# xieydd/crane-scheduler

Measured on AMD Instinct MI355X. Metric: placements/sec, higher is better.
Workload: dtype f64

## Files before the change

### crane-scheduler_amd/crane_dyn/__init__.py

```python
from __future__ import annotations

import ctypes as C
import os

import numpy as np

_HERE = os.path.dirname(os.path.abspath(__file__))
LIB_PATH = os.path.join(os.path.dirname(_HERE), "lib", "libcrane_dyn.so")

CRANE_TS_INVALID = -(2**63)
CRANE_POD_DAEMONSET = 1
_ERRS = {-1: "invalid argument", -2: "HIP error", -3: "bad state", -4: "policy parse error", -5: "I/O error"}


class CraneError(RuntimeError):
    def __init__(self, code, msg):
        super().__init__(f"{_ERRS.get(code, code)}: {msg}")
        self.code = code


class _CPolicy(C.Structure):
    _fields_ = [
        ("n_sync", C.c_int32), ("sync_name", C.POINTER(C.c_char_p)), ("sync_period_ns", C.POINTER(C.c_int64)),
        ("n_pred", C.c_int32), ("pred_name", C.POINTER(C.c_char_p)), ("pred_limit", C.POINTER(C.c_double)),
# ... 74 lines not shown
        "crane_dyn_group_set_option": (C.c_int, [vp, C.c_char_p, C.c_int64]),
        "crane_dyn_group_size": (C.c_int32, [vp]),
        "crane_dyn_group_shard": (C.c_int, [vp, C.c_int32, P(C.c_int32), P(C.c_int64), P(C.c_int64)]),
        "crane_dyn_group_engine": (vp, [vp, C.c_int32, C.c_int32]),
        "crane_dyn_group_upload_nodes": (C.c_int, [vp, C.c_int64, vp, vp, vp, vp]),
        "crane_dyn_group_upload_bindings": (C.c_int, [vp, C.c_int64, vp, vp]),
        "crane_dyn_group_step_keys_async": (C.c_int, [vp, C.c_int64, C.c_int64, C.c_int64, vp, vp, vp]),
        "crane_dyn_group_sync": (C.c_int, [vp]),
        "crane_dyn_group_schedule": (C.c_int, [vp, C.c_int64, C.c_int64, C.c_int64, vp, vp, vp, vp]),
        "crane_dyn_group_step_keys_batch": (C.c_int, [vp, C.c_int32, vp, vp, C.c_int64, vp, vp, vp]),
        "crane_dyn_group_update_nodes": (C.c_int, [vp, C.c_int64, vp, vp, vp, vp, vp]),
        "crane_dyn_group_update_node_steps": (C.c_int, [vp, C.c_int64, vp, vp, vp, vp, vp, C.c_int64, C.c_int64,
                                                        vp, vp, vp, vp]),
        "crane_dyn_group_resize_nodes": (C.c_int, [vp, C.c_int64]),
        "crane_dyn_group_binding_records": (C.c_int, [vp, C.c_int64, C.c_int64]),
        "crane_dyn_group_add_bindings": (C.c_int, [vp, C.c_int64, vp, vp]),
        "crane_dyn_group_gc_bindings": (C.c_int, [vp, C.c_int64]),
        "crane_dyn_group_binding_count": (C.c_int64, [vp]),
        "crane_dyn_group_refresh_hot_values": (C.c_int, [vp, C.c_int64, C.c_int64]),
        "crane_dyn_group_hot_values": (C.c_int, [vp, C.c_int64, vp]),
        "crane_dyn_group_node_steps": (C.c_int, [vp, C.c_int64, C.c_int64, C.c_int64, vp, vp, vp, vp]),
        "crane_queue_create": (C.c_int, [C.c_int32, C.c_int32, P(vp)]),
        "crane_queue_wait": (C.c_int, [vp]),
        "crane_queue_last_error": (C.c_char_p, [vp]),
        "crane_queue_packets": (C.c_uint64, [vp]),
        "crane_queue_destroy": (C.c_int, [vp]),
        "crane_dyn_step_keys_queue": (C.c_int, [vp, C.c_int64, C.c_int64, C.c_int64, vp, vp, vp, vp]),
        "crane_dyn_forget_queue": (C.c_int, [vp, vp]),
        "crane_dyn_step_flush": (C.c_int, [vp]),
        "crane_dyn_num_predicates": (C.c_int32, [vp]),
        "crane_dyn_filter_counts_async": (C.c_int, [vp, C.c_int64, vp, vp, vp, vp]),
        "crane_dyn_filter_counts": (C.c_int, [vp, C.c_int64, vp, vp, vp]),
        "crane_dyn_group_filter_counts": (C.c_int, [vp, C.c_int64, vp, vp, vp]),
    }
    for name, (res, args) in sig.items():
        f = getattr(L, name)
        f.restype = res
        f.argtypes = args
    return L


lib = _load()

ABI_SYMBOLS = (
    "crane_policy_load_file", "crane_policy_load_bytes", "crane_policy_view", "crane_policy_free",
    "crane_tz_offset", "crane_parse_annotation", "crane_parse_annotations", "crane_dyn_create", "crane_dyn_destroy", "crane_dyn_last_error",
    "crane_dyn_num_metrics", "crane_dyn_metric_name", "crane_dyn_upload_nodes", "crane_dyn_upload_bindings",
    "crane_dyn_refresh_hot_values", "crane_dyn_eval", "crane_dyn_eval_keys_async", "crane_dyn_step_keys_async",
    "crane_dyn_refresh_hot_values_async", "crane_dyn_node_pass_async", "crane_dyn_greedy", "crane_dyn_key_node",
    "crane_dyn_set_profiling", "crane_dyn_stage_times", "crane_dyn_hot_values",
    "crane_dyn_version", "crane_dyn_binding_records", "crane_dyn_add_bindings", "crane_dyn_gc_bindings",
    "crane_dyn_binding_count", "crane_dyn_eval_compact", "crane_dyn_eval_matrix_async", "crane_dyn_set_option",
    "crane_translate_event", "crane_dyn_debug_trace", "crane_num_feasible_nodes_to_find", "crane_dyn_select",
    "crane_tz_load", "crane_tz_load_bytes", "crane_tz_free", "crane_tz_lookup", "crane_tz_date",
    "crane_parse_annotation_tz", "crane_parse_annotations_tz", "crane_dyn_step_slots", "crane_dyn_node_steps",
    "crane_dyn_node_steps_subset", "crane_dyn_update_nodes", "crane_dyn_update_node_steps",
    "crane_dyn_forget_stream", "crane_dyn_resize_nodes", "crane_shard_range", "crane_dyn_group_create", "crane_dyn_group_destroy",
    "crane_dyn_group_last_error", "crane_dyn_group_set_option", "crane_dyn_group_size", "crane_dyn_group_shard",
    "crane_dyn_group_engine", "crane_dyn_group_upload_nodes", "crane_dyn_group_upload_bindings",
    "crane_dyn_group_step_keys_async", "crane_dyn_group_sync", "crane_dyn_group_schedule",
    "crane_dyn_group_step_keys_batch", "crane_dyn_group_update_nodes", "crane_dyn_group_update_node_steps",
    "crane_dyn_group_resize_nodes", "crane_dyn_group_binding_records", "crane_dyn_group_add_bindings",
    "crane_dyn_group_gc_bindings", "crane_dyn_group_binding_count", "crane_dyn_group_refresh_hot_values",
    "crane_dyn_group_hot_values", "crane_dyn_group_node_steps",
    "crane_queue_create", "crane_queue_wait", "crane_queue_last_error", "crane_queue_destroy",
    "crane_queue_packets",
    "crane_dyn_step_keys_queue", "crane_dyn_forget_queue", "crane_dyn_step_flush",
    "crane_dyn_num_predicates", "crane_dyn_filter_counts_async", "crane_dyn_filter_counts",
    "crane_dyn_group_filter_counts",
)


def _ptr(a):
    return None if a is None else C.c_void_p(a.ctypes.data)


def num_feasible_nodes_to_find(n_nodes, percentage=0):
    return lib.crane_num_feasible_nodes_to_find(int(n_nodes), int(percentage))


class Policy:

    def __init__(self, spec):
        self.spec = {k: [tuple(x) for x in spec.get(k, [])] for k in ("syncPolicy", "predicate", "priority", "hotValue")}
        sp, pr, pi, hv = (self.spec[k] for k in ("syncPolicy", "predicate", "priority", "hotValue"))
        n = lambda xs: max(1, len(xs))
        self._keep = [
            (C.c_char_p * n(sp))(*[a.encode() for a, _ in sp]), (C.c_int64 * n(sp))(*[int(b) for _, b in sp]),
            (C.c_char_p * n(pr))(*[a.encode() for a, _ in pr]), (C.c_double * n(pr))(*[float(b) for _, b in pr]),
            (C.c_char_p * n(pi))(*[a.encode() for a, _ in pi]), (C.c_double * n(pi))(*[float(b) for _, b in pi]),
            (C.c_int64 * n(hv))(*[int(a) for a, _ in hv]), (C.c_int64 * n(hv))(*[int(b) for _, b in hv]),
        ]
        k = self._keep
        cp = C.POINTER
        self.c = _CPolicy(len(sp), C.cast(k[0], cp(C.c_char_p)), C.cast(k[1], cp(C.c_int64)),
                          len(pr), C.cast(k[2], cp(C.c_char_p)), C.cast(k[3], cp(C.c_double)),
                          len(pi), C.cast(k[4], cp(C.c_char_p)), C.cast(k[5], cp(C.c_double)),
                          len(hv), C.cast(k[6], cp(C.c_int64)), C.cast(k[7], cp(C.c_int64)))

    @staticmethod
    def _from_doc(doc):
        v = lib.crane_policy_view(doc).contents
# ... 6 lines not shown
        lib.crane_policy_free(doc)
        return Policy(spec)

    @staticmethod
    def load_bytes(data: bytes | str) -> "Policy":
        if isinstance(data, str):
            data = data.encode()
        doc, err = C.c_void_p(), C.create_string_buffer(512)
        rc = lib.crane_policy_load_bytes(data, len(data), C.byref(doc), err, len(err))
        if rc:
            raise CraneError(rc, err.value.decode())
        return Policy._from_doc(doc)

    @staticmethod
    def load_file(path: str) -> "Policy":
        doc, err = C.c_void_p(), C.create_string_buffer(512)
        rc = lib.crane_policy_load_file(path.encode(), C.byref(doc), err, len(err))
        if rc:
            raise CraneError(rc, err.value.decode())
        return Policy._from_doc(doc)


def default_policy_spec():
    m = 60 * 10**9
    return {
        "syncPolicy": [("cpu_usage_avg_5m", 3 * m), ("cpu_usage_max_avg_1h", 15 * m), ("cpu_usage_max_avg_1d", 180 * m),
                       ("mem_usage_avg_5m", 3 * m), ("mem_usage_max_avg_1h", 15 * m), ("mem_usage_max_avg_1d", 180 * m)],
        "predicate": [("cpu_usage_avg_5m", 0.65), ("cpu_usage_max_avg_1h", 0.75), ("mem_usage_avg_5m", 0.65),
                      ("mem_usage_max_avg_1h", 0.75)],
        "priority": [("cpu_usage_avg_5m", 0.2), ("cpu_usage_max_avg_1h", 0.3), ("cpu_usage_max_avg_1d", 0.5),
                     ("mem_usage_avg_5m", 0.2), ("mem_usage_max_avg_1h", 0.3), ("mem_usage_max_avg_1d", 0.5)],
        "hotValue": [(5 * m, 5), (1 * m, 2)],
    }


def tz_offset(name: str | None = None) -> int:
    off = C.c_int64()
    rc = lib.crane_tz_offset(None if name is None else name.encode(), C.byref(off))
    if rc:
        raise CraneError(rc, f"unsupported time zone {name!r}")
    return off.value


def parse_annotation(s: str, tz_offset_s: int):
    b = s.encode()
    v, t = C.c_double(), C.c_int64()
    lib.crane_parse_annotation(b, len(b), tz_offset_s, C.byref(v), C.byref(t))
    return v.value, t.value


class Zone:

    def __init__(self, name=None, zoneinfo_dir=None, tzif=None):
        h = C.c_void_p()
        if tzif is not None:
            rc = lib.crane_tz_load_bytes(tzif, len(tzif), C.byref(h))
        else:
            rc = lib.crane_tz_load((name or "").encode(), None if zoneinfo_dir is None else zoneinfo_dir.encode(),
                                   C.byref(h))
        if rc:
            raise CraneError(rc, f"time zone {name!r} not loadable")
        self.h = h

    def lookup(self, unix_s):
        off, st, en = C.c_int32(), C.c_int64(), C.c_int64()
        lib.crane_tz_lookup(self.h, int(unix_s), C.byref(off), C.byref(st), C.byref(en))
# ... 624 lines not shown
```

### crane-scheduler_amd/csrc/engine.hip

```cpp
#include <hip/hip_runtime.h>

#include <algorithm>
#include <chrono>
#include <cmath>
#include <cstdio>
#include <cstdlib>
#include <cstring>
#include <memory>
#include <mutex>
#include <string>
#include <vector>

#include "../../include/crane_dyn.h"
#include "bindings.hpp"
#include "dyn_types.hpp"
#include "kernels.hpp"

using namespace crane;

namespace {

hipError_t before_free() { return crane::tl_aql ? crane::aql_wait(crane::tl_aql) : hipSuccess; }

template <typename T>
// ... 594 lines not shown
        HIPTRY(h, launch_hot_count_large(rp.bn, h->sd->bts.p, rp.Bk, h->N, cut, gl, h->k2_sorted.p, h->buckets.p,
                                         h->n_cu, st, kK2lThreads));
        h->buckets_zero = false;
        h->buckets_dense = true;
        return CRANE_OK;
    }
    h->buckets_dense = false;
    if (!h->buckets_zero)
        if (int rc = zero_for(h, h->buckets.p, nb, st)) return rc;
    HIPTRY(h, launch_hot_count(h->sd->bnode.p, h->sd->bts.p, h->B, h->N, rp.cut, h->buckets.p, st));
    h->buckets_zero = false;
    return CRANE_OK;
}

static int hot_values_locked(crane_dyn* h, int64_t now_ns, int64_t hv_ts_ns, hipStream_t st,
                             const PodPrep* pods = nullptr, bool* pods_done = nullptr) {
    if (pods_done) *pods_done = false;
    RefreshPlan rp;
    if (int rc = refresh_plan(h, now_ns, hv_ts_ns, st, rp)) return rc;
    return refresh_launch(h, rp, st, pods, pods_done);
}

static int k1_bs(const crane_dyn* h) {
    return h->hv_from_counts && h->counts_pending && h->hx_pending ? 1 << h->hx_g.bb : kK1Block;
}

static int k1_args(crane_dyn* h, K1Args& a, uint32_t* cnt_out, const K1Step* step, bool* consume_out) {
    if (h->N < 0) return h->fail(CRANE_E_STATE, "upload nodes before the node pass");
    a = K1Args{};
    a.pol = h->dp;
    a.N = h->N;
    a.val = h->sd->val.p;
    a.ts = h->sd->ts.p;
    const bool keep = !step;
    a.out = keep ? h->rec.p : nullptr;
    a.hv_ts_counts = h->hv_ts_counts;
    const bool consume = h->hv_from_counts && h->counts_pending;
    if (cnt_out && !consume) return h->fail(CRANE_E_STATE, "per-window counts need a hot-value refresh first");
    if (consume) {
        HIPTRY(h, h->hvc.reserve((size_t)std::max<int64_t>(h->N, 1)));
        if (h->hx_pending) {
            const HotPart& g = h->hx_g;
            a.hx_region = h->k2_sorted.p;
            a.hx_CO = h->k2_sorted.p + g.cap;
            a.hx_nblk = g.nblk;
        } else if (h->dl_pending) {
            a.buckets = h->dl_adj[h->dl_cur].p;
            a.bucket_base = h->dl_zero ? h->dl_adj[h->dl_cur].p : h->dl_base.p;
            a.buckets_keep = 0;
        } else {
            a.buckets = h->buckets.p;
            a.buckets_keep = h->buckets_dense ? 1 : 0;
        }
        a.cnt_out = cnt_out;
        a.hvc_out = h->hvc.p;
    } else if (h->hv_from_counts) {
        a.hv = h->hvc.p;
    } else if (h->have_hv) {
        a.hv = h->sd->hv.p;
        a.hv_ts = h->sd->hv_ts.p;
    }
    a.threads = k1_bs(h);
    a.trace = (h->N + a.threads - 1) / a.threads <= kTraceWgs ? h->trace_region(1) : nullptr;
    *consume_out = consume;
    return CRANE_OK;
}
// ... 426 lines not shown
    Options& o = h->opt;
    auto range = [&](int64_t lo, int64_t hi) { return value >= lo && value <= hi; };
    if (n == "diag_slices" && range(0, 0x7FFFFFFF)) {
        o.diag_slices = (int)value;
        return CRANE_OK;
    }
    if (n == "k2_form" && (value == 0 || value == 2 || value == 3)) o.k2_form = (int)value;
    else if (n == "keys_path" && range(0, 1)) o.keys_path = (int)value;
    else if (n == "greedy_form" && range(0, 1)) o.greedy_form = (int)value;
    else if (n == "sel_chain" && range(0, 1)) o.sel_chain = (int)value;
    else if (n == "step_rows" && range(0, 1)) o.step_rows = (int)value;
    else if (n == "step_pieces" && range(0, 2)) o.step_pieces = (int)value;
    else if (n == "step_lds_cap" && value >= 0) o.step_lds_cap = (int)std::min<int64_t>(value, 1 << 30);
    else if (n == "k2_sorted" && range(0, 1)) o.k2_sorted = (int)value;
    else if (n == "k2_delta" && range(0, 1)) o.k2_delta = (int)value;
    else if (n == "step_defer" && range(0, 2)) o.step_defer = (int)value;
    else if (n == "k1_stream" && range(0, 1)) o.k1_stream = (int)value;
    else if (n == "k1_tail" && (value == 0 || value == 1 || value == 4)) o.k1_tail = (int)value;
    else if (n == "trace" && range(0, 1)) {
        o.trace = value != 0;
        if (o.trace) {
            hipError_t e = hipSetDevice(h->device);
            if (e == hipSuccess) e = h->trace.reserve((size_t)3 * kTraceWgs * 8);
            if (e == hipSuccess) e = hipMemsetAsync(h->trace.p, 0, sizeof(unsigned long long) * h->trace.n, h->stream);
            if (e == hipSuccess) e = hipStreamSynchronize(h->stream);
            if (e != hipSuccess) return h->hipfail(e, "trace buffer");
        }
    }
    else return h->fail(CRANE_E_INVALID, "unknown option or value: " + n + "=" + std::to_string(value));
    h->rec_dirty = true;
    return CRANE_OK;
}

int64_t crane_dyn_debug_trace(crane_dyn* h, int32_t which, int64_t max, uint64_t* out) {
    if (!h || which < 0 || which > 2 || max < 0 || (max > 0 && !out)) return CRANE_E_INVALID;
    std::lock_guard<std::mutex> g(h->mu);
    if (!h->opt.trace || !h->trace.p) return h->fail(CRANE_E_STATE, "option \"trace\" is off");
    const int64_t n = std::min<int64_t>(max, kTraceWgs * 8);
    HIPTRY(h, hipSetDevice(h->device));
    HIPTRY(h, hipStreamSynchronize(h->stream));
    HIPTRY(h, hipDeviceSynchronize());
    HIPTRY(h, hipMemcpy(out, h->trace_region(which), sizeof(uint64_t) * n, hipMemcpyDeviceToHost));
    return n;
}

int crane_dyn_upload_nodes(crane_dyn* h, int64_t n, int64_t node_offset, const double* val, const int64_t* ts,
                           const double* hv, const int64_t* hv_ts) {
    if (!h) return CRANE_E_INVALID;
    Locked lk(h);
    if (lk.rc) return lk.rc;
    if (h->N == -2) return h->fail(CRANE_E_STATE, "engine was not created successfully");
    if (n < 0 || n > 0xFFFFFFFFLL || node_offset < 0 || node_offset + n > 0xFFFFFFFFLL)
        return h->fail(CRANE_E_INVALID, "node count/offset out of range (global indices must fit 32 bits)");
    const int64_t M = h->dp.n_slots;
    if (n > 0 && M > 0 && (!val || !ts)) return h->fail(CRANE_E_INVALID, "val/ts must not be NULL");
    if ((hv == nullptr) != (hv_ts == nullptr)) return h->fail(CRANE_E_INVALID, "hv and hv_ts must both be set or NULL");
    HIPTRY(h, hipSetDevice(h->device));
    if (int rc = quiesce(h)) return rc;
    HIPTRY(h, h->sd->val.reserve((size_t)(M * n)));
    HIPTRY(h, h->sd->ts.reserve((size_t)(M * n)));
    HIPTRY(h, h->sd->hv.reserve((size_t)n));
    HIPTRY(h, h->sd->hv_ts.reserve((size_t)n));
    HIPTRY(h, h->rec.reserve((size_t)n * h->rec_bytes));
    if (M * n > 0) {
        HIPTRY(h, hipMemcpyAsync(h->sd->val.p, val, sizeof(double) * M * n, hipMemcpyHostToDevice, h->stream));
        HIPTRY(h, hipMemcpyAsync(h->sd->ts.p, ts, sizeof(int64_t) * M * n, hipMemcpyHostToDevice, h->stream));
// ... 987 lines not shown
```

### crane-scheduler_amd/csrc/k1stream.hip

```cpp
#include <hip/hip_runtime.h>

#include "k1stream_body.hpp"

namespace crane {

template <int PD, int PR, bool FULL>
__global__ __launch_bounds__(256) __attribute__((amdgpu_waves_per_eu(PD * PR <= 24 ? K1S_WAVES : 1)))
void k1_stream_steps(K1Args a, K1Step step) {
    __shared__ K1Lds<PD, PR> lds;
    k1_stream_body<PD, PR, FULL, (int)sizeof(K1Args) + (int)sizeof(K1Step)>(a, step, blockIdx.x, gridDim.x, lds);
}

template <int PD, int PR, bool FULL = false>
static hipError_t launch_t(const K1Args& a, const K1Step& sa, hipStream_t st) {
    const unsigned grid = (unsigned)((a.N + 255) / 256);
    return klaunch("k1_stream_steps", k1_stream_steps<PD, PR, FULL>, dim3(grid), dim3(256), 0, st, a, sa);
}

hipError_t launch_stream_steps(int pd, int pr, const K1Args& a, const K1Step& sa, hipStream_t st) {
    if (a.N <= 0) return hipSuccess;
    if (K1S_FULL && a.pol.npd == 4 && a.pol.npr == 6 && a.pol.n_win == kFullWin) return launch_t<4, 6, true>(a, sa, st);
    if (pd <= 4 && pr <= 6) return launch_t<4, 6>(a, sa, st);
    if (pd <= 8 && pr <= 8) return launch_t<8, 8>(a, sa, st);
    return launch_t<16, 16>(a, sa, st);
}

}
```

### crane-scheduler_amd/csrc/k1stream_body.hpp

```cpp
#pragma once
#include <hip/hip_runtime.h>

#include <cstddef>

#include "dyn_types.hpp"
#include "kernels.hpp"
#include "node_rec.hpp"
#include "step_node.hpp"

namespace crane {

#ifndef K1S_SKIP
#define K1S_SKIP 0
#endif
#ifndef K1S_TAIL1
#define K1S_TAIL1 1
#endif
#ifndef K1S_WAVES
#define K1S_WAVES 7
#endif
#ifndef K1S_KWARM
#define K1S_KWARM 1
#endif
#ifndef K1S_FULL
// ... 135 lines not shown
    const int T0 = ONE ? 0 : __builtin_amdgcn_readfirstlane((int)(threadIdx.x >> 6));
    const int tl = lane < 32 ? lane : 64;
    int32_t n[NK], fl[NK];
    Step1 r[NK];
    SmallScan sc[NK];
#pragma unroll
    for (int k = 0; k < NK; ++k) {
        const int T = T0 + k;
        n[k] = __builtin_amdgcn_readfirstlane(T ? n1 : n0);
        fl[k] = block_flat_max<256>(ssh, T);
        r[k].bp = 0;
        r[k].k0 = r[k].k1 = -1;
        if (lane < n[k]) r[k] = s1l[T * kSCap + lane];
    }
#pragma unroll
    for (int k = 0; k < NK; ++k) sc[k] = small_scan(r[k], n[k], lane < 32 ? r[k].bp : pre[k], tl);
#pragma unroll
    for (int k = 0; k < NK; ++k) small_records_store(T0 + k, n[k], r[k], sc[k], st, blk);
    CRANE_TSTAMP(trace, wg, 6);
    if (rows) {
#pragma unroll
        for (int k = 0; k < NK; ++k) small_row_store(T0 + k, 0, sc[k], fl[k], st, blk);
        for (int t0 = 16; t0 < st.ntiles; t0 += 16) {
#pragma unroll
            for (int k = 0; k < NK; ++k) {
                const SmallScan s = small_scan(r[k], n[k], small_tile_bound(st, T0 + k, t0, lane), 64);
                small_row_store(T0 + k, t0, s, fl[k], st, blk);
            }
        }
    }
    CRANE_TSTAMP(trace, wg, 4);
}

constexpr int kFullWin = 2;
template <int PD, int PR>
struct K1Lds {
    alignas(16) NodeRec<PD, PR> lrec[kSRec];
    alignas(16) Step1 s1l[2 * kSCap];
    alignas(16) Step1 srt[2 * kSCap];
    alignas(16) uint32_t xch[5][4];
    StepShared ssh;
    uint8_t rank_lane[256];
};
template <int PD, int PR, bool FULL, int WARM>
__device__ __forceinline__ void k1_stream_body(const K1Args& a, const K1Step& step, const int64_t wg, const int64_t nwg,
                                               K1Lds<PD, PR>& lds) {
    using Rec = NodeRec<PD, PR>;
    constexpr int BS = 256;
    const int npd = FULL ? PD : a.pol.npd, npr = FULL ? PR : a.pol.npr, nwin = FULL ? kFullWin : a.pol.n_win;
    Rec* const lrec = lds.lrec;
    uint8_t* const rank_lane = lds.rank_lane;
    Step1* const s1l = lds.s1l;
    Step1* const srt = lds.srt;
    uint32_t(*const xch)[4] = lds.xch;
    StepShared& ssh = lds.ssh;
    const DevPolicy& pol = a.pol;
    const int64_t N = a.N;
    const int64_t blk = xcd_block(wg, nwg), first = blk * BS, n = first + threadIdx.x;
    CRANE_TSTAMP(a.trace, wg, 0);
    const int lo = (int)min((int64_t)threadIdx.x, N - 1 - first);
    const int64_t bt0 = step.batch[0], bt1 = step.batch[1];
    int64_t pt[PD], qt[PR];
    double pv[PD], qv[PR];
#pragma unroll
    for (int k = 0; k < PD; ++k) {
        pt[k] = kTsInvalid;
        pv[k] = 0.0;
    }
#pragma unroll
    for (int k = 0; k < PR; ++k) {
        qt[k] = kTsInvalid;
        qv[k] = 0.0;
    }
    if (FULL || pol.n_slots > 0) {
#pragma unroll
        for (int k = 0; k < PD; ++k) {
            const int64_t row = k < npd ? pol.pred_slot[k] : 0;
            pt[k] = (a.ts + (row * N + first))[lo];
            pv[k] = (a.val + (row * N + first))[lo];
        }
#pragma unroll
        for (int k = 0; k < PR; ++k) {
            const int64_t row = k < npr ? pol.prio_slot[k] : 0;
            qt[k] = (a.ts + (row * N + first))[lo];
            qv[k] = (a.val + (row * N + first))[lo];
        }
    }
    uint32_t bc[kMaxWin];
    double hvl = 0.0;
    int64_t hvt = kTsInvalid;
    if (a.buckets) {
        const uint32_t* __restrict__ base = a.bucket_base ? a.bucket_base : a.buckets;
        uint32_t bz[kMaxWin];
#pragma unroll
        for (int b = 0; b < kMaxWin; ++b) {
            bc[b] = b < nwin ? (a.buckets + first)[(int64_t)b * N + lo] : 0u;
            bz[b] = b < nwin ? (base + first)[(int64_t)b * N + lo] : 0u;
        }
        if (a.bucket_base) bucket_anchor_counts(bz, bc);
    } else if (a.hv) {
        hvl = a.hv[first + lo];
        hvt = a.hv_ts ? a.hv_ts[first + lo] : a.hv_ts_counts;
    }
#if K1S_KWARM
    kernarg_warm<WARM>();
#endif
    const int64_t tmin = readfirstlane64(bt0), tmax = readfirstlane64(bt1);
    if (threadIdx.x < 4) ssh.lc[threadIdx.x >> 1][threadIdx.x & 1] = 0;
    CRANE_TSTAMP(a.trace, wg, 1);
    const bool valid = n < N;
    int64_t e_fail = kTsInvalid;
#pragma unroll
    for (int k = 0; k < PD; ++k) {
        const double u = pv[k], lim = pol.pred_limit[k];
        const int64_t e = sat_add(pt[k], pol.pred_dur[k]);
        const bool over = k < npd && pt[k] != kTsInvalid && !(u < 0.0) && lim != 0.0 && u > lim;
        e_fail = over ? max(e_fail, e) : e_fail;
    }
    Rec hr;
    if (a.buckets) {
        if (valid && !a.buckets_keep) {
#pragma unroll
            for (int b = 0; b < kMaxWin; ++b)
                if (b < nwin) (a.buckets + first)[(int64_t)b * N + threadIdx.x] = 0;
        }
        rec_hot_counts<PD, PR, FULL ? kFullWin : 0>(pol, bc, N, n, valid ? a.cnt_out : nullptr, valid ? a.hvc_out : nullptr,
                               a.hv_ts_counts, hr);
    } else if (a.hv) {
        rec_hot_annotation<PD, PR>(hvl, hvt, hr);
    } else {
        hr.pen = 0;
        hr.e_hv = kTsInvalid;
    }
    double s = 0.0;
    StepRange both;
    int64_t ep[PR];
    double tp[PR];
#pragma unroll
    for (int k = 0; k < PR; ++k) {
        const bool use = k < npr && qt[k] != kTsInvalid && !(qv[k] < 0.0);
        double term = (1.0 - qv[k]) * pol.prio_w[k];
        term = term * 100.0;
        const int64_t e = sat_add(qt[k], pol.prio_dur[k]);
        ep[k] = use ? e : kTsInvalid;
        tp[k] = use ? term : 0.0;
        s = tmin < ep[k] ? s + tp[k] : s;
        both.add(ep[k], tmin, tmax);
    }
    both.add(hr.e_hv, tmin, tmax);
    const int32_t s0 = score_of_sum(s, tmin < hr.e_hv ? hr.pen : 0, step.wsum, step.noprio, step.winv);
    StepRange g[2];
    StepSlots so;
    step_classify(both, e_fail, valid, s0, n, tmin, tmax, g, so);
    CRANE_TSTAMP(a.trace, wg, 2);
    const int lane = threadIdx.x & 63, wv = threadIdx.x >> 6;
    const uint32_t w0 = g[0].word(), w1 = g[1].word(), w2 = (g[0].cnt | g[1].cnt) ? 1u : 0u;
    uint32_t e0 = wave_scan_add(w0), e1 = wave_scan_add(w1), e2 = wave_scan_add(w2);
    const int32_t fm0 = wave_max(so.flat0), fm1 = wave_max(so.flat1);
    if (lane == 0) {
        ssh.fm[0][wv] = fm0;
        ssh.fm[1][wv] = fm1;
    }
    if (lane == 63) {
        xch[0][wv] = e0;
        xch[1][wv] = e1;
        xch[2][wv] = e2;
    }
    e0 -= w0;
    e1 -= w1;
    e2 -= w2;
    __syncthreads();
    uint32_t base[3], tot[3];
#pragma unroll
    for (int k = 0; k < 3; ++k) {
        const uint4 x = *reinterpret_cast<const uint4*>(xch[k]);
        base[k] = (wv > 0 ? x.x : 0u) + (wv > 1 ? x.y : 0u) + (wv > 2 ? x.z : 0u);
        tot[k] = x.x + x.y + x.z + x.w;
// ... 103 lines not shown
```

### crane-scheduler_amd/csrc/kernels.hpp

```cpp
#pragma once
#include <hip/hip_ext.h>
#include <hip/hip_runtime.h>
#include <stdint.h>

#include "aql.hpp"
#include "dyn_types.hpp"

namespace crane {

enum { kShape4x6 = 0, kShape8x8 = 1, kShape16x16 = 2 };

struct KernelTimer {
    virtual ~KernelTimer() = default;
    virtual void next(const char* name, hipEvent_t* start, hipEvent_t* stop) = 0;
};
extern thread_local KernelTimer* tl_ktimer;

template <typename... KArgs, typename... Args>
inline hipError_t klaunch(const char* name, void (*kernel)(KArgs...), dim3 grid, dim3 block, size_t lds,
                          hipStream_t st, Args... args) {
    if (tl_aql) {
        static_assert((sizeof(KArgs) + ... + 0) + 16 * sizeof...(KArgs) <= kAqlMaxArgs, "kernel arguments too large");
        alignas(16) unsigned char buf[kAqlMaxArgs];
        size_t off = 0;
// ... 253 lines not shown
    int64_t reset_P;
    const int32_t* bnode;
    int64_t N;
    const HotDelta* d;
    uint32_t* adj;
    const PodPrep* pods;
};
bool step_one_has(int shape);
constexpr int kStepOneDeltaChunk = 512;
int64_t step_one_workgroups(int64_t nk3s, int64_t N_k1, int64_t ntiles, int64_t delta_len);
extern const int kStepOneWgPerCu;
hipError_t launch_step_one(const StepOne& s, hipStream_t st);
hipError_t launch_keys_reset(long long* keys, int64_t P, hipStream_t st);
hipError_t launch_step_pods(const int64_t* now, const uint8_t* flags, int64_t P, long long* keys, int64_t* batch,
                            int64_t* batch_next,
                            const StepGeometry& g, int32_t* perm, int64_t* pnow, int64_t* tile_mm, hipStream_t s);
hipError_t launch_step_nodes(int shape, const void* rec, int64_t N, double wsum, int32_t noprio,
                             const StepTables& st, const StepGeometry& g, const int64_t* tile_mm, hipStream_t s);
hipError_t launch_step_pairs(const K3sBatch& b, hipStream_t s);
struct K1Step {
    const int64_t* tile_mm;
    const int64_t* batch;
    int32_t ntiles;
    int32_t noprio;
    double wsum;
    double winv;
    StepTables st;
    void* srec;
    int32_t tail1;
};

size_t node_rec_bytes(int shape);

struct K1Args {
    DevPolicy pol;
    int64_t N;
    const double* val;
    const int64_t* ts;
    const double* hv;
    const int64_t* hv_ts;
    uint32_t* buckets;
    const uint32_t* bucket_base;
    int32_t buckets_keep;
    int64_t hv_ts_counts;
    void* out;
    uint32_t* cnt_out;
    double* hvc_out;
    const uint32_t* hx_region;
    const uint32_t* hx_CO;
    int32_t hx_nblk;
    int32_t threads;
    unsigned long long* trace;
};
hipError_t launch_node_pass(int shape, const K1Args& a, hipStream_t st, const K1Step* step = nullptr,
                            int stream = 0);
hipError_t launch_stream_steps(int pd, int pr, const K1Args& a, const K1Step& sa, hipStream_t st);

}
```

### crane-scheduler_amd/csrc/step.hip

```cpp
#include <hip/hip_runtime.h>

#include <algorithm>

#include "dyn_types.hpp"
#include "kernels.hpp"
#include "pods.hpp"
#include "lds_hash.hpp"
#include "step_node.hpp"
#include "k1stream_body.hpp"

#ifndef K3S_BUCKETS
#define K3S_BUCKETS 1
#endif
#ifndef K3_KWARM
#define K3_KWARM 1
#endif

namespace crane {

constexpr int kPodTile = 1024;

__global__ __launch_bounds__(kPodTile) void k3p_pods(PodPrep pp) {
    extern __shared__ __attribute__((aligned(16))) unsigned char lds[];
    k3p_tile<kPodTile>(blockIdx.x, pp, lds);
// ... 576 lines not shown
    return klaunch("k3s_eval+k2_delta+k3p_pods", k3s_delta_pods, dim3((unsigned)grid), dim3(kK3sThreads), lds, s, k,
                   (int32_t)nk, bnode, N, d, adj, pp);
}

bool step_one_has(int shape) { return shape == kShape4x6; }

int64_t step_one_workgroups(int64_t nk3s, int64_t N_k1, int64_t ntiles, int64_t delta_len) {
    const int64_t nk1 = (N_k1 + 255) / 256;
    return nk3s + (nk1 + 7) / 8 * 8 + 2 * ntiles + (delta_len + kStepOneDeltaChunk - 1) / kStepOneDeltaChunk;
}

hipError_t launch_step_one(const StepOne& s, hipStream_t st) {
    const bool k3s = s.k3s && s.k3s->P > 0 && s.k3s->N > 0, k1 = s.k1 && s.ks && s.k1->N > 0;
    const bool delta = s.d != nullptr, pods = s.pods && s.pods->P > 0;
    if (delta && (s.d->n_win < 1 || s.d->n_win > kDeltaMaxWin || s.d->n_rng < 0 || s.d->n_rng > kMaxWin ||
                  s.N >= (1LL << 27)))
        return hipErrorInvalidValue;
    if (k1 && (s.k1->threads != 256 || s.k1->out || s.k1->hx_region || !s.ks->st.stage)) return hipErrorInvalidValue;
    const int64_t nk = k3s ? s.k3s->g.ngroups * s.k3s->g.R : 0;
    const int64_t nk1 = k1 ? (s.k1->N + 255) / 256 : 0, nk1pad = (nk1 + 7) / 8 * 8;
    const int64_t L = delta && s.d->n_rng > 0 ? s.d->start[s.d->n_rng] : 0;
    const KeyReset kr{s.reset_keys, k1 && s.reset_keys && s.reset_P > 0 ? s.reset_P : 0};
    const int64_t nreset = (kr.P + kResetPerWg - 1) / kResetPerWg;
    const int64_t grid = nk + nk1pad + nreset + (pods ? s.pods->ntiles : 0) +
                         (L + kStepOneDeltaChunk - 1) / kStepOneDeltaChunk;
    if (grid >= (1LL << 31)) return hipErrorInvalidValue;
    if (grid == 0) return hipSuccess;
    const K3sBatch kb = k3s ? *s.k3s : K3sBatch{};
    const K3sArgs k{kb.st, kb.perm, kb.pnow, kb.tile_mm, kb.P, kb.node_offset, kb.g.R, kb.keys};
    const K1Args a = k1 ? *s.k1 : K1Args{};
    const K1Step ks = k1 ? *s.ks : K1Step{};
    const HotDelta d = delta ? *s.d : HotDelta{};
    const PodPrep pp = pods ? *s.pods : PodPrep{};
    const bool full = K1S_FULL && k1 && a.pol.npd == 4 && a.pol.npr == 6 && a.pol.n_win == kFullWin;
    static const hipError_t attr[2] = {
        hipFuncSetAttribute((const void*)step_one_launch<false>, hipFuncAttributeMaxDynamicSharedMemorySize,
                            (int)kStepOneLds),
        hipFuncSetAttribute((const void*)step_one_launch<true>, hipFuncAttributeMaxDynamicSharedMemorySize,
                            (int)kStepOneLds)};
    if (attr[full] != hipSuccess) return attr[full];
    const char* nm = "k3s_eval+k1_stream_steps+k2_delta+k3p_pods";
    return full ? klaunch(nm, step_one_launch<true>, dim3((unsigned)grid), dim3(kStepOneThreads), kStepOneLds, st, k,
                          (int32_t)nk, (int32_t)nk1, (int32_t)nk1pad, (int32_t)nreset, kr, a, ks, s.bnode, s.N, d, s.adj, pp)
                : klaunch(nm, step_one_launch<false>, dim3((unsigned)grid), dim3(kStepOneThreads), kStepOneLds, st, k,
                          (int32_t)nk, (int32_t)nk1, (int32_t)nk1pad, (int32_t)nreset, kr, a, ks, s.bnode, s.N, d, s.adj, pp);
}

hipError_t launch_keys_reset(long long* keys, int64_t P, hipStream_t st) {
    if (P <= 0 || !keys) return hipSuccess;
    return klaunch("keys_reset", keys_reset, dim3((unsigned)((P + 255) / 256)), dim3(256), 0, st, keys, P);
}

hipError_t launch_step_pairs(const K3sBatch& b, hipStream_t s) {
    if (b.P <= 0 || b.N <= 0) return hipSuccess;
    const dim3 grid((unsigned)(b.g.ngroups * b.g.R)), blk(kK3sThreads);
    return klaunch("k3s_eval", k3s_eval, grid, blk, 0, s, b.st, b.perm, b.pnow, b.tile_mm, b.P, b.node_offset, b.g.R,
                   b.keys);
}

}
```

### include/crane_dyn.h

```cpp
#ifndef CRANE_DYN_H
#define CRANE_DYN_H
#include <stddef.h>
#include <stdint.h>

#ifdef __cplusplus
extern "C" {
#endif

#define CRANE_OK 0
#define CRANE_E_INVALID -1
#define CRANE_E_HIP -2
#define CRANE_E_STATE -3
#define CRANE_E_PARSE -4
#define CRANE_E_IO -5

#define CRANE_TS_INVALID INT64_MIN

#define CRANE_POD_DAEMONSET 1u

typedef struct crane_policy {
    int32_t n_sync;
    const char *const *sync_name;
    const int64_t *sync_period_ns;
    int32_t n_pred;
// ... 81 lines not shown
int crane_dyn_select(crane_dyn *h, int64_t n_pods, const int64_t *d_now_ns, const uint8_t *d_pod_flags,
                     const uint8_t *d_ext_ok, const int64_t *d_ext_score, int64_t dyn_weight, int32_t percentage,
                     int64_t start, uint64_t tie_seed, int64_t *d_chosen, int64_t *d_total, int64_t *d_wstart,
                     int64_t *d_wlen, int64_t *next_start, void *stream);

int crane_dyn_eval_keys_async(crane_dyn *h, int64_t n_pods, const int64_t *d_now_ns,
                              const uint8_t *d_pod_flags, int64_t *d_keys, void *stream);
int crane_dyn_step_keys_async(crane_dyn *h, int64_t now_ns, int64_t hv_ts_ns, int64_t n_pods,
                              const int64_t *d_now_ns, const uint8_t *d_pod_flags, int64_t *d_keys, void *stream);
typedef struct crane_queue crane_queue;
int crane_queue_create(int32_t device, int32_t ring_kind, crane_queue **out);
int crane_queue_wait(crane_queue *q);
const char *crane_queue_last_error(const crane_queue *q);
uint64_t crane_queue_packets(const crane_queue *q);
int crane_queue_destroy(crane_queue *q);
int crane_dyn_step_keys_queue(crane_dyn *h, int64_t now_ns, int64_t hv_ts_ns, int64_t n_pods,
                              const int64_t *d_now_ns, const uint8_t *d_pod_flags, int64_t *d_keys, crane_queue *q);
int crane_dyn_step_flush(crane_dyn *h);
int crane_dyn_forget_queue(crane_dyn *h, crane_queue *q);
int crane_dyn_refresh_hot_values_async(crane_dyn *h, int64_t now_ns, int64_t hv_ts_ns, void *stream);
int crane_dyn_node_pass_async(crane_dyn *h, void *stream);

int crane_dyn_set_profiling(crane_dyn *h, int on);
int crane_dyn_stage_times(crane_dyn *h, int32_t max, const char **names, double *ms);

int crane_dyn_greedy(crane_dyn *h, int64_t n_pods, int64_t now_ns, const uint8_t *pod_flags, int64_t *chosen);

int64_t crane_dyn_key_node(int64_t key, int64_t *score);

const char *crane_dyn_version(void);

int crane_dyn_set_option(crane_dyn *h, const char *name, int64_t value);
int64_t crane_dyn_debug_trace(crane_dyn *h, int32_t which, int64_t max, uint64_t *out);

typedef struct crane_dyn_group crane_dyn_group;
int crane_shard_range(int64_t n_nodes, int32_t n_shards, int32_t shard, int64_t *lo, int64_t *hi);
int crane_dyn_group_create(const crane_policy *pol, int32_t n_dev, const int32_t *devices, int32_t depth,
                           crane_dyn_group **out);
int crane_dyn_group_destroy(crane_dyn_group *g);
const char *crane_dyn_group_last_error(const crane_dyn_group *g);
int crane_dyn_group_set_option(crane_dyn_group *g, const char *name, int64_t value);
int32_t crane_dyn_group_size(const crane_dyn_group *g);
int crane_dyn_group_shard(const crane_dyn_group *g, int32_t i, int32_t *device, int64_t *lo, int64_t *hi);
crane_dyn *crane_dyn_group_engine(crane_dyn_group *g, int32_t i, int32_t slot);
int crane_dyn_group_upload_nodes(crane_dyn_group *g, int64_t n_nodes, const double *val, const int64_t *ts,
                                 const double *hv, const int64_t *hv_ts);
int crane_dyn_group_upload_bindings(crane_dyn_group *g, int64_t n, const int32_t *node, const int64_t *ts_s);
int crane_dyn_group_step_keys_async(crane_dyn_group *g, int64_t now_ns, int64_t hv_ts_ns, int64_t n_pods,
                                    const int64_t *const *d_now, const uint8_t *const *d_flags,
                                    int64_t *const *d_keys);
int crane_dyn_group_step_keys_batch(crane_dyn_group *g, int32_t n_batches, const int64_t *now_ns,
                                    const int64_t *hv_ts_ns, int64_t n_pods, const int64_t *const *d_now,
                                    const uint8_t *const *d_flags, int64_t *const *d_keys);
int crane_dyn_group_sync(crane_dyn_group *g);
int crane_dyn_group_update_nodes(crane_dyn_group *g, int64_t k, const int64_t *idx, const double *val,
                                 const int64_t *ts, const double *hv, const int64_t *hv_ts);
int crane_dyn_group_update_node_steps(crane_dyn_group *g, int64_t k, const int64_t *idx, const double *val,
                                      const int64_t *ts, const double *hv, const int64_t *hv_ts, int64_t t0_ns,
                                      int64_t t1_ns, uint8_t *n_steps, int64_t *bp, int8_t *first_fail,
                                      int8_t *score);
int crane_dyn_group_resize_nodes(crane_dyn_group *g, int64_t n);
int crane_dyn_group_binding_records(crane_dyn_group *g, int64_t size, int64_t gc_time_range_ns);
int crane_dyn_group_add_bindings(crane_dyn_group *g, int64_t n, const int32_t *node, const int64_t *ts_s);
int crane_dyn_group_gc_bindings(crane_dyn_group *g, int64_t now_ns);
int64_t crane_dyn_group_binding_count(crane_dyn_group *g);
int crane_dyn_group_refresh_hot_values(crane_dyn_group *g, int64_t now_ns, int64_t hv_ts_ns);
// ... 18 lines not shown
```

Baseline: 2.396 billion.

## Alias predicate rows onto priority rows in the full-policy node kernel

In the specialised full-policy path, predicate metric rows that match a priority row with the same duration are no longer loaded separately. Their values, timestamps and expiry times are reused from the priority loads through a fixed alias pattern, and row offsets are precomputed on the host. Loads use a scalar-base address helper meant to give cheaper global addressing. The full path is now gated on the policy actually matching the alias pattern, which also adds a correctness check, and new ABI functions expose the alias map.

```diff
diff --git a/crane-scheduler_amd/crane_dyn/__init__.py b/crane-scheduler_amd/crane_dyn/__init__.py
--- a/crane-scheduler_amd/crane_dyn/__init__.py
+++ b/crane-scheduler_amd/crane_dyn/__init__.py
@@ -130,6 +130,8 @@
         "crane_dyn_filter_counts_async": (C.c_int, [vp, C.c_int64, vp, vp, vp, vp]),
         "crane_dyn_filter_counts": (C.c_int, [vp, C.c_int64, vp, vp, vp]),
         "crane_dyn_group_filter_counts": (C.c_int, [vp, C.c_int64, vp, vp, vp]),
+        "crane_dyn_k1_alias": (C.c_int32, [vp, C.c_int32, P(C.c_int32), P(C.c_int32)]),
+        "crane_k1_alias_rows": (C.c_int, [C.c_int32, vp, vp, C.c_int32, vp, vp, vp]),
     }
     for name, (res, args) in sig.items():
         f = getattr(L, name)
@@ -165,7 +167,7 @@
     "crane_queue_packets",
     "crane_dyn_step_keys_queue", "crane_dyn_forget_queue", "crane_dyn_step_flush",
     "crane_dyn_num_predicates", "crane_dyn_filter_counts_async", "crane_dyn_filter_counts",
-    "crane_dyn_group_filter_counts",
+    "crane_dyn_group_filter_counts", "crane_dyn_k1_alias", "crane_k1_alias_rows",
 )
 
 
@@ -238,6 +240,32 @@
                      ("mem_usage_avg_5m", 0.2), ("mem_usage_max_avg_1h", 0.3), ("mem_usage_max_avg_1d", 0.5)],
         "hotValue": [(5 * m, 5), (1 * m, 2)],
     }
+
+
+def k1_alias(policy: Policy):
+    h = C.c_void_p()
+    rc = lib.crane_dyn_create(C.byref(policy.c), 0, C.byref(h))
+    try:
+        if rc == -1:
+            raise CraneError(rc, lib.crane_dyn_last_error(h).decode() if h.value else "")
+        out, n = (C.c_int32 * 16)(), C.c_int32()
+        full = lib.crane_dyn_k1_alias(h, 16, out, C.byref(n))
+        return list(out)[:n.value], bool(full)
+    finally:
+        if h.value:
+            lib.crane_dyn_destroy(h)
+
+
+def k1_alias_rows(pred_row, pred_dur_ns, prio_row, prio_dur_ns):
+    pr, pd = np.ascontiguousarray(pred_row, np.int32), np.ascontiguousarray(pred_dur_ns, np.int64)
+    qr, qd = np.ascontiguousarray(prio_row, np.int32), np.ascontiguousarray(prio_dur_ns, np.int64)
+    if pr.shape != pd.shape or qr.shape != qd.shape or pr.ndim != 1 or qr.ndim != 1:
+        raise ValueError("one row and one duration per term")
+    out = np.empty(len(pr), np.int32)
+    rc = lib.crane_k1_alias_rows(len(pr), _ptr(pr), _ptr(pd), len(qr), _ptr(qr), _ptr(qd), _ptr(out))
+    if rc:
+        raise CraneError(rc, "crane_k1_alias_rows")
+    return out.tolist()
 
 
 def tz_offset(name: str | None = None) -> int:
diff --git a/crane-scheduler_amd/csrc/engine.hip b/crane-scheduler_amd/csrc/engine.hip
--- a/crane-scheduler_amd/csrc/engine.hip
+++ b/crane-scheduler_amd/csrc/engine.hip
@@ -650,6 +650,7 @@
     a.N = h->N;
     a.val = h->sd->val.p;
     a.ts = h->sd->ts.p;
+    k1_row_offsets(a);
     const bool keep = !step;
     a.out = keep ? h->rec.p : nullptr;
     a.hv_ts_counts = h->hv_ts_counts;
@@ -1142,6 +1143,24 @@
     return CRANE_OK;
 }
 
+int crane_k1_alias_rows(int32_t n_pred, const int32_t* pred_row, const int64_t* pred_dur_ns, int32_t n_prio,
+                        const int32_t* prio_row, const int64_t* prio_dur_ns, int32_t* alias) {
+    if (n_pred < 0 || n_prio < 0 || (n_pred > 0 && (!pred_row || !pred_dur_ns || !alias)) ||
+        (n_prio > 0 && (!prio_row || !prio_dur_ns)))
+        return CRANE_E_INVALID;
+    k1_alias_rows(n_pred, pred_row, pred_dur_ns, n_prio, prio_row, prio_dur_ns, alias);
+    return CRANE_OK;
+}
+
+int32_t crane_dyn_k1_alias(const crane_dyn* h, int32_t max, int32_t* alias, int32_t* n_active) {
+    if (!h || max < 0 || (max > 0 && !alias)) return CRANE_E_INVALID;
+    int32_t m[kMaxPred];
+    k1_alias_map(h->dp, m);
+    if (n_active) *n_active = h->dp.npd;
+    for (int32_t k = 0; k < max; ++k) alias[k] = k < kMaxPred ? m[k] : -1;
+    return k1_full_policy(h->dp) ? 1 : 0;
+}
+
 int64_t crane_dyn_debug_trace(crane_dyn* h, int32_t which, int64_t max, uint64_t* out) {
     if (!h || which < 0 || which > 2 || max < 0 || (max > 0 && !out)) return CRANE_E_INVALID;
     std::lock_guard<std::mutex> g(h->mu);
diff --git a/crane-scheduler_amd/csrc/k1stream.hip b/crane-scheduler_amd/csrc/k1stream.hip
--- a/crane-scheduler_amd/csrc/k1stream.hip
+++ b/crane-scheduler_amd/csrc/k1stream.hip
@@ -19,7 +19,7 @@
 
 hipError_t launch_stream_steps(int pd, int pr, const K1Args& a, const K1Step& sa, hipStream_t st) {
     if (a.N <= 0) return hipSuccess;
-    if (K1S_FULL && a.pol.npd == 4 && a.pol.npr == 6 && a.pol.n_win == kFullWin) return launch_t<4, 6, true>(a, sa, st);
+    if (K1S_FULL && k1_full_policy(a.pol)) return launch_t<kFullPred, kFullPrio, true>(a, sa, st);
     if (pd <= 4 && pr <= 6) return launch_t<4, 6>(a, sa, st);
     if (pd <= 8 && pr <= 8) return launch_t<8, 8>(a, sa, st);
     return launch_t<16, 16>(a, sa, st);
diff --git a/crane-scheduler_amd/csrc/k1stream_body.hpp b/crane-scheduler_amd/csrc/k1stream_body.hpp
--- a/crane-scheduler_amd/csrc/k1stream_body.hpp
+++ b/crane-scheduler_amd/csrc/k1stream_body.hpp
@@ -191,7 +191,13 @@
     CRANE_TSTAMP(trace, wg, 4);
 }
 
-constexpr int kFullWin = 2;
+template <class T>
+__device__ __forceinline__ T ld_lane(const T* p, uint32_t i) {
+    uint64_t base = reinterpret_cast<uint64_t>(p);
+    asm("" : "+s"(base));
+    using G = const __attribute__((address_space(1))) char*;
+    return *(const __attribute__((address_space(1))) T*)((G)base + i * (uint32_t)sizeof(T));
+}
 template <int PD, int PR>
 struct K1Lds {
     alignas(16) NodeRec<PD, PR> lrec[kSRec];
@@ -231,7 +237,15 @@
         qt[k] = kTsInvalid;
         qv[k] = 0.0;
     }
-    if (FULL || pol.n_slots > 0) {
+    if constexpr (FULL) {
+        static_assert(!FULL || (PD == kFullPred && PR == kFullPrio), "the alias pattern's shape");
+#pragma unroll
+        for (int k = 0; k < PR; ++k) {
+            const int64_t off = a.prio_off[k] + first;
+            qt[k] = ld_lane(a.ts + off, (uint32_t)lo);
+            qv[k] = ld_lane(a.val + off, (uint32_t)lo);
+        }
+    } else if (pol.n_slots > 0) {
 #pragma unroll
         for (int k = 0; k < PD; ++k) {
             const int64_t row = k < npd ? pol.pred_slot[k] : 0;
@@ -253,8 +267,13 @@
         uint32_t bz[kMaxWin];
 #pragma unroll
         for (int b = 0; b < kMaxWin; ++b) {
-            bc[b] = b < nwin ? (a.buckets + first)[(int64_t)b * N + lo] : 0u;
-            bz[b] = b < nwin ? (base + first)[(int64_t)b * N + lo] : 0u;
+            if constexpr (FULL) {
+                bc[b] = b < nwin ? ld_lane(a.buckets + first + (int64_t)b * N, (uint32_t)lo) : 0u;
+                bz[b] = b < nwin ? ld_lane(base + first + (int64_t)b * N, (uint32_t)lo) : 0u;
+            } else {
+                bc[b] = b < nwin ? (a.buckets + first)[(int64_t)b * N + lo] : 0u;
+                bz[b] = b < nwin ? (base + first)[(int64_t)b * N + lo] : 0u;
+            }
         }
         if (a.bucket_base) bucket_anchor_counts(bz, bc);
     } else if (a.hv) {
@@ -269,10 +288,27 @@
     CRANE_TSTAMP(a.trace, wg, 1);
     const bool valid = n < N;
     int64_t e_fail = kTsInvalid;
+    int64_t eq[PR], pe[PD];
+#pragma unroll
+    for (int k = 0; k < PR; ++k) eq[k] = sat_add(qt[k], pol.prio_dur[k]);
+    if constexpr (FULL) {
+        const int64_t at[PD] = {qt[kFullAlias[0]], qt[kFullAlias[1]], qt[kFullAlias[2]], qt[kFullAlias[3]]};
+        const double av[PD] = {qv[kFullAlias[0]], qv[kFullAlias[1]], qv[kFullAlias[2]], qv[kFullAlias[3]]};
+        const int64_t ae[PD] = {eq[kFullAlias[0]], eq[kFullAlias[1]], eq[kFullAlias[2]], eq[kFullAlias[3]]};
+#pragma unroll
+        for (int k = 0; k < PD; ++k) {
+            pt[k] = at[k];
+            pv[k] = av[k];
+            pe[k] = ae[k];
+        }
+    } else {
+#pragma unroll
+        for (int k = 0; k < PD; ++k) pe[k] = sat_add(pt[k], pol.pred_dur[k]);
+    }
 #pragma unroll
     for (int k = 0; k < PD; ++k) {
         const double u = pv[k], lim = pol.pred_limit[k];
-        const int64_t e = sat_add(pt[k], pol.pred_dur[k]);
+        const int64_t e = pe[k];
         const bool over = k < npd && pt[k] != kTsInvalid && !(u < 0.0) && lim != 0.0 && u > lim;
         e_fail = over ? max(e_fail, e) : e_fail;
     }
@@ -300,8 +336,7 @@
         const bool use = k < npr && qt[k] != kTsInvalid && !(qv[k] < 0.0);
         double term = (1.0 - qv[k]) * pol.prio_w[k];
         term = term * 100.0;
-        const int64_t e = sat_add(qt[k], pol.prio_dur[k]);
-        ep[k] = use ? e : kTsInvalid;
+        ep[k] = use ? eq[k] : kTsInvalid;
         tp[k] = use ? term : 0.0;
         s = tmin < ep[k] ? s + tp[k] : s;
         both.add(ep[k], tmin, tmax);
diff --git a/crane-scheduler_amd/csrc/kernels.hpp b/crane-scheduler_amd/csrc/kernels.hpp
--- a/crane-scheduler_amd/csrc/kernels.hpp
+++ b/crane-scheduler_amd/csrc/kernels.hpp
@@ -309,6 +309,29 @@
 
 size_t node_rec_bytes(int shape);
 
+constexpr int kFullPred = 4, kFullPrio = 6, kFullWin = 2;
+constexpr int32_t kFullAlias[kFullPred] = {0, 1, 3, 4};
+inline void k1_alias_rows(int npd, const int32_t* pred_slot, const int64_t* pred_dur, int npr, const int32_t* prio_slot,
+                          const int64_t* prio_dur, int32_t* alias) {
+    for (int k = 0; k < npd; ++k) {
+        alias[k] = -1;
+        for (int j = 0; j < npr && alias[k] < 0; ++j)
+            if (pred_slot[k] == prio_slot[j] && pred_dur[k] == prio_dur[j]) alias[k] = j;
+    }
+}
+inline void k1_alias_map(const DevPolicy& p, int32_t (&alias)[kMaxPred]) {
+    for (int k = 0; k < kMaxPred; ++k) alias[k] = -1;
+    k1_alias_rows(p.npd, p.pred_slot, p.pred_dur, p.npr, p.prio_slot, p.prio_dur, alias);
+}
+inline bool k1_full_policy(const DevPolicy& p) {
+    if (p.npd != kFullPred || p.npr != kFullPrio || p.n_win != kFullWin) return false;
+    int32_t alias[kMaxPred];
+    k1_alias_map(p, alias);
+    for (int k = 0; k < kFullPred; ++k)
+        if (alias[k] != kFullAlias[k]) return false;
+    return true;
+}
+
 struct K1Args {
     DevPolicy pol;
     int64_t N;
@@ -328,7 +351,11 @@
     int32_t hx_nblk;
     int32_t threads;
     unsigned long long* trace;
-};
+    int64_t prio_off[kFullPrio];
+};
+inline void k1_row_offsets(K1Args& a) {
+    for (int k = 0; k < kFullPrio; ++k) a.prio_off[k] = k < a.pol.npr ? (int64_t)a.pol.prio_slot[k] * a.N : 0;
+}
 hipError_t launch_node_pass(int shape, const K1Args& a, hipStream_t st, const K1Step* step = nullptr,
                             int stream = 0);
 hipError_t launch_stream_steps(int pd, int pr, const K1Args& a, const K1Step& sa, hipStream_t st);
diff --git a/crane-scheduler_amd/csrc/step.hip b/crane-scheduler_amd/csrc/step.hip
--- a/crane-scheduler_amd/csrc/step.hip
+++ b/crane-scheduler_amd/csrc/step.hip
@@ -632,7 +632,7 @@
     const K1Step ks = k1 ? *s.ks : K1Step{};
     const HotDelta d = delta ? *s.d : HotDelta{};
     const PodPrep pp = pods ? *s.pods : PodPrep{};
-    const bool full = K1S_FULL && k1 && a.pol.npd == 4 && a.pol.npr == 6 && a.pol.n_win == kFullWin;
+    const bool full = K1S_FULL && k1 && k1_full_policy(a.pol);
     static const hipError_t attr[2] = {
         hipFuncSetAttribute((const void*)step_one_launch<false>, hipFuncAttributeMaxDynamicSharedMemorySize,
                             (int)kStepOneLds),
diff --git a/include/crane_dyn.h b/include/crane_dyn.h
--- a/include/crane_dyn.h
+++ b/include/crane_dyn.h
@@ -137,6 +137,9 @@
 
 int crane_dyn_set_option(crane_dyn *h, const char *name, int64_t value);
 int64_t crane_dyn_debug_trace(crane_dyn *h, int32_t which, int64_t max, uint64_t *out);
+int32_t crane_dyn_k1_alias(const crane_dyn *h, int32_t max, int32_t *alias, int32_t *n_active);
+int crane_k1_alias_rows(int32_t n_pred, const int32_t *pred_row, const int64_t *pred_dur_ns, int32_t n_prio,
+                        const int32_t *prio_row, const int64_t *prio_dur_ns, int32_t *alias);
 
 typedef struct crane_dyn_group crane_dyn_group;
 int crane_shard_range(int64_t n_nodes, int32_t n_shards, int32_t shard, int64_t *lo, int64_t *hi);
```

Result: no change. 2.413 billion (median of 6 runs) (+0.7%).
